# zpelgrims/pota

Hardware: AMD Instinct MI355X
Metric: bidir redistribution Msamples/s at 4K, double-gauss 50mm (higher is better)
Workload: dtype f64

## Files before the change

pota_amd/csrc/lentil_device.h:

```cpp
#pragma once
#include <hip/hip_runtime.h>
#include <stdint.h>

#include "../../include/lentil_hip.h"

#define LD_DEV __device__ __forceinline__

namespace lentil {

constexpr float kAiPi = 3.14159265358979323846f;
constexpr float kAiPiOver2 = 1.57079632679489661923f;
constexpr float kAiEpsilon = 1.0e-4f;
constexpr float kAiInfinite = 1.0e30f;
constexpr double kPi = 3.14159265358979323846;

enum PolyId {
  P_OUT_X = 0, P_OUT_Y, P_OUT_DX, P_OUT_DY, P_OUT_T,
  P_AP_X, P_AP_Y, P_AP_DX, P_AP_DY,
  P_DAP_00, P_DAP_01, P_DAP_10, P_DAP_11,
  P_DOUT_00, P_DOUT_01, P_DOUT_10, P_DOUT_11,
  P_DAPPOS_00, P_DAPPOS_01, P_DAPPOS_10, P_DAPPOS_11,
  P_COUNT
};

// ... 220 lines not shown
  ody = vx * ey0 + vy * ey1 + vz * ey2;
}

LD_DEV double ipow_u(double x, uint32_t e) {
  uint32_t odd = 0, n = 0;
  while (e > 2) { odd = (odd << 1) | (e & 1u); ++n; e >>= 1; }
  double p = (e == 2) ? x * x : x;
  for (uint32_t i = 0; i < n; ++i) {
    p = (odd & 1u) ? (x * p) * p : p * p;
    odd >>= 1;
  }
  return p;
}

struct LdsLens {
  const DevTerm *terms;
  const DevLens *k;

  LD_DEV double eval(int pid, const double v[4]) const {
    const uint32_t first = k->first[pid], count = k->count[pid];
    double sum = 0.0;
    for (uint32_t i = 0; i < count; ++i) {
      const DevTerm t = terms[first + i];
      const uint32_t e = __builtin_amdgcn_readfirstlane(t.e);
      double term = t.c;
#pragma unroll
      for (int var = 0; var < 4; ++var) {
        const uint32_t ev = (e >> (4 * var)) & 15u;
        if (ev == 1) term = term * v[var];
        else if (ev > 1) term = term * ipow_u(v[var], ev);
      }
      const uint32_t el = (e >> 16) & 15u;
      if (el) term = term * k->lambda_pow[el];
      sum = (i == 0) ? term : sum + term;
    }
    return sum;
  }

  LD_DEV void eval_bw(const double v[4], double pred_ap[2], double Jap[4], double out[4], double Jout[4]) const {
    pred_ap[0] = eval(P_AP_X, v);
    pred_ap[1] = eval(P_AP_Y, v);
    Jap[0] = eval(P_DAP_00, v); Jap[1] = eval(P_DAP_01, v);
    Jap[2] = eval(P_DAP_10, v); Jap[3] = eval(P_DAP_11, v);
    out[0] = eval(P_OUT_X, v); out[1] = eval(P_OUT_Y, v);
    out[2] = eval(P_OUT_DX, v); out[3] = eval(P_OUT_DY, v);
    Jout[0] = eval(P_DOUT_00, v); Jout[1] = eval(P_DOUT_01, v);
    Jout[2] = eval(P_DOUT_10, v); Jout[3] = eval(P_DOUT_11, v);
  }
  LD_DEV double transmittance(const double v[4]) const { return eval(P_OUT_T, v); }
  LD_DEV void eval_fw_newton(const double v[4], double pred_ap[2], double pred_dir[2], double Jap[4], double Jappos[4]) const {
    pred_ap[0] = eval(P_AP_X, v); pred_ap[1] = eval(P_AP_Y, v);
    pred_dir[0] = eval(P_AP_DX, v); pred_dir[1] = eval(P_AP_DY, v);
    Jap[0] = eval(P_DAP_00, v); Jappos[0] = eval(P_DAPPOS_00, v);
    Jap[1] = eval(P_DAP_01, v); Jappos[1] = eval(P_DAPPOS_01, v);
    Jap[2] = eval(P_DAP_10, v); Jappos[2] = eval(P_DAPPOS_10, v);
    Jap[3] = eval(P_DAP_11, v); Jappos[3] = eval(P_DAPPOS_11, v);
  }
  LD_DEV void eval_out(const double v[4], double out[4]) const {
    out[0] = eval(P_OUT_X, v); out[1] = eval(P_OUT_Y, v);
    out[2] = eval(P_OUT_DX, v); out[3] = eval(P_OUT_DY, v);
  }
  LD_DEV const DevLens &consts() const { return *k; }
};

struct NewtonState {
  double x, y, dx, dy;
  double sqr_err, sqr_ap_err;
  double out[4];
  int k, error;
};

LD_DEV void newton_init(NewtonState &s) {
  s.x = 0; s.y = 0; s.dx = 0; s.dy = 0;
  s.sqr_err = 1e30; s.sqr_ap_err = 1e30;
  s.out[0] = s.out[1] = s.out[2] = s.out[3] = 0.0;
  s.k = 0; s.error = 0;
}

LD_DEV bool newton_continue(const NewtonState &s) {
  const double eps = 1e-8;
  return s.k < 100 && (s.sqr_err > eps || s.sqr_ap_err > eps) && s.error == 0;
}

template <class Lens>
LD_DEV void newton_iter(const Lens &L, const double scene[3], double ap_x, double ap_y, NewtonState &s) {
  const DevLens &k = L.consts();
  const double R = k.outer_pupil_curvature_radius;
  const double prev_sqr_err = s.sqr_err, prev_sqr_ap_err = s.sqr_ap_err;
  const double begin[4] = {s.x, s.y, s.dx, s.dy};
  double pred_ap[2], Jap[4], Jout[4];
  L.eval_bw(begin, pred_ap, Jap, s.out, Jout);
  const double d0 = ap_x - pred_ap[0], d1 = ap_y - pred_ap[1];
  s.sqr_ap_err = d0 * d0 + d1 * d1;
  {
    const double invdet = 1.0 / (Jap[0] * Jap[3] - Jap[1] * Jap[2]);
    const double i00 = Jap[3] * invdet, i11 = Jap[0] * invdet;
    const double i01 = -Jap[1] * invdet, i10 = -Jap[2] * invdet;
    s.dx += i00 * d0; s.dy += i10 * d0;
    s.dx += i01 * d1; s.dy += i11 * d1;
  }
  double pos[3], dir[3];
  double on_dx, on_dy;
  if (k.outer_pupil_geometry == LENTIL_GEOM_SPHERICAL) {
    sphereToCs(s.out[0], s.out[1], s.out[2], s.out[3], pos, dir, -R, R);
    double vx = scene[0] - pos[0], vy = scene[1] - pos[1], vz = scene[2] - pos[2];
    normalise3(vx, vy, vz);
    csToSphere(pos, vx, vy, vz, on_dx, on_dy, -R, R);
  } else {
    const bool cy = k.outer_pupil_geometry == LENTIL_GEOM_CYL_Y;
    cylinderToCs(s.out[0], s.out[1], s.out[2], s.out[3], pos, dir, -R, R, cy);
    double vx = scene[0] - pos[0], vy = scene[1] - pos[1], vz = scene[2] - pos[2];
    normalise3(vx, vy, vz);
    csToCylinder(pos, vx, vy, vz, on_dx, on_dy, -R, R, cy);
  }
  const double e0 = on_dx - s.out[2], e1 = on_dy - s.out[3];
  s.sqr_err = e0 * e0 + e1 * e1;
  {
    const double invdet = 1.0 / (Jout[0] * Jout[3] - Jout[1] * Jout[2]);
    const double i00 = Jout[3] * invdet, i11 = Jout[0] * invdet;
    const double i01 = -Jout[1] * invdet, i10 = -Jout[2] * invdet;
    s.x += 0.72 * i00 * e0; s.y += 0.72 * i10 * e0;
    s.x += 0.72 * i01 * e1; s.y += 0.72 * i11 * e1;
  }
  int error = s.error;
  if (s.sqr_err > prev_sqr_err) error |= 1;
  if (s.sqr_ap_err > prev_sqr_ap_err) error |= 2;
  if (s.out[0] != s.out[0]) error |= 4;
  if (s.out[2] * s.out[2] + s.out[3] * s.out[3] > 1.0) error |= 8;
  if (s.k < 10) error = 0;
  s.error = error;
  s.k += 1;
}

template <class Lens>
LD_DEV double lens_evaluate(const Lens &L, const double in[4], double out[4]) {
  L.eval_out(in, out);
  return fmax(0.0, L.transmittance(in));
}

template <class Lens>
LD_DEV void lens_pt_sample_aperture(const Lens &L, double in[4], double ap_x, double ap_y, double dist,
                                    double &out_dx, double &out_dy) {
  double dx = in[2], dy = in[3];
  double pred_dx = 0.0, pred_dy = 0.0;
  double sqr_err = 3.4028234663852886e38;
  for (int k = 0; k < 5 && sqr_err > 1e-4; ++k) {
    const double begin[4] = {in[0] + dist * dx, in[1] + dist * dy, dx, dy};
    double pred[2], pred_dir[2], Jap[4], Jappos[4];
    L.eval_fw_newton(begin, pred, pred_dir, Jap, Jappos);
    const double pred_x = pred[0], pred_y = pred[1];
    pred_dx = pred_dir[0];
    pred_dy = pred_dir[1];
    const double j00 = Jap[0] + dist * Jappos[0];
    const double j01 = Jap[1] + dist * Jappos[1];
    const double j10 = Jap[2] + dist * Jappos[2];
    const double j11 = Jap[3] + dist * Jappos[3];
    const double invdet = 1.0 / (j00 * j11 - j01 * j10);
    const double i00 = j11 * invdet, i11 = j00 * invdet, i01 = -j01 * invdet, i10 = -j10 * invdet;
    const double r0 = ap_x - pred_x, r1 = ap_y - pred_y;
    dx += i00 * r0; dy += i10 * r0;
    dx += i01 * r1; dy += i11 * r1;
    sqr_err = r0 * r0 + r1 * r1;
  }
  out_dx = pred_dx; out_dy = pred_dy;
  in[2] = dx; in[3] = dy;
}

LD_DEV double y0_plane_z(const double pos[3], const double dir[3]) {
  const double n = sqrt(dir[0] * dir[0] + dir[1] * dir[1] + dir[2] * dir[2]);
  const double dy = dir[1] / n, dz = dir[2] / n;
  return pos[2] + (dz * (0.0 - pos[1])) / dy;
}

template <class Lens>
LD_DEV double camera_get_y0_intersection_distance(const Lens &L, double sensor_shift, double aperture_housing_radius,
                                                  double sensor_out[4], double out[4], double &transmittance) {
  const DevLens &k = L.consts();
  double sensor[4] = {0.0, 0.0, 0.0, 0.0};
  double adx, ady;
  lens_pt_sample_aperture(L, sensor, 0.0, aperture_housing_radius * 0.25, sensor_shift, adx, ady);
  sensor[0] += sensor[2] * sensor_shift;
  sensor[1] += sensor[3] * sensor_shift;
  transmittance = lens_evaluate(L, sensor, out);
  for (int c = 0; c < 4; ++c) sensor_out[c] = sensor[c];
  const double R = k.outer_pupil_curvature_radius;
  double pos[3], dir[3];
  if (k.outer_pupil_geometry == LENTIL_GEOM_SPHERICAL) sphereToCs(out[0], out[1], out[2], out[3], pos, dir, -R, R);
  else cylinderToCs(out[0], out[1], out[2], out[3], pos, dir, -R, R, k.outer_pupil_geometry == LENTIL_GEOM_CYL_Y);
  return y0_plane_z(pos, dir);
}

template <class Lens>
LD_DEV double newton_finish(const Lens &L, const NewtonState &s, double &out4) {
  const DevLens &k = L.consts();
  int error = s.error;
  if (s.out[0] * s.out[0] + s.out[1] * s.out[1] > k.outer_pupil_radius * k.outer_pupil_radius) error |= 16;
  if (error == 0) {
    const double begin[4] = {s.x, s.y, s.dx, s.dy};
    out4 = L.transmittance(begin);
  } else {
    out4 = 0.0;
  }
  return fmax(0.0, out4);
}

template <class Lens>
LD_DEV double lt_sample_aperture(const Lens &L, const double scene[3], double ap_x, double ap_y,
                                 double sensor[4], double out[5], int *iters = nullptr) {
  NewtonState s;
  newton_init(s);
  while (newton_continue(s)) newton_iter(L, scene, ap_x, ap_y, s);
  const double T = newton_finish(L, s, out[4]);
  out[0] = s.out[0]; out[1] = s.out[1]; out[2] = s.out[2]; out[3] = s.out[3];
  if (iters) *iters = s.k;
// ... 466 lines not shown
```

pota_amd/csrc/lentil_hip.hip:

```cpp
#include <hip/hip_runtime.h>
#include <hip/hip_ext.h>

#include <algorithm>
#include <atomic>
#include <chrono>
#include <cmath>
#include <cstdio>
#include <cstdlib>
#include <cstring>
#include <deque>
#include <mutex>
#include <new>
#include <string>
#include <vector>

#include "lentil_kernels.h"
#include "lentil_closest_replay.h"
#include "lentil_tl_chroma_mgpu.h"
#include "lentil_lens_jit.h"
#include "lentil_camera_rays.h"
#include "lentil_trace_points.h"
#include "lentil_list_draws.h"
#include "generated/embedded_sources.inc"

// ... 2615 lines not shown
    const int rc = redistribute_streamed(ctx, &streamed, &deferred);
    if (rc) return rc;
    if (ctx->stall_redo) return LENTIL_OK;
  }
  if (!streamed) { const int rc = join_clear(ctx); if (rc) return rc; }
  if (!streamed && ctx->V.n) {
    ScanPlan plan;
    {
      const int rc = plan_scan(ctx, plan);
      if (rc) return rc;
    }
    const uint32_t M = plan.M;
    for (int ci = 0; ci < C; ++ci) {
      lentil_hip_ctx::Chunk &ch = ctx->chunks[ci];
      if (M) {
        auto bound = [&](int i) -> uint64_t {
          if (i <= 0) return 0;
          if (i >= C) return plan.n_tiles;
          const double f0 = C > 1 ? ctx->first_chunk_frac : 1.0;
          const double x = f0 + (1.0 - f0) * (double)(i - 1) / (double)(C - 1);
          const uint64_t b = (uint64_t)((double)plan.n_tiles * x);
          return b > plan.n_tiles ? plan.n_tiles : b;
        };
        ch.tile_begin = bound(ci);
        ch.tile_end = bound(ci + 1);
        ch.v_begin = ch.tile_begin * plan.sa.ppt * M;
        ch.v_end = ch.tile_end * plan.sa.ppt * M;
        if (ch.v_begin > ctx->V.n) ch.v_begin = ctx->V.n;
        if (ch.v_end > ctx->V.n) ch.v_end = ctx->V.n;
      } else {
        ch.v_begin = ((ctx->V.n * ci / C) + 63) & ~63ull;
        ch.v_end = ci == C - 1 ? ctx->V.n : (((ctx->V.n * (ci + 1) / C) + 63) & ~63ull);
        if (ch.v_begin > ctx->V.n) ch.v_begin = ctx->V.n;
        if (ch.v_end > ctx->V.n) ch.v_end = ctx->V.n;
      }
      if (ch.v_end > ch.v_begin) {
        const int rc = launch_scan(ctx, plan, ch, ctx->d_ctr + ci);
        if (rc) return rc;
        ++ctx->last_scan_launches;
      }
      HIP_TRY(ctx, hipEventRecord(ch.scanned, ctx->stream));
    }
  }
  if (!streamed) {
    HIP_TRY(ctx, hipEventRecord(ctx->ev[1], ctx->stream));
    HIP_TRY(ctx, hipEventRecord(ctx->scans_done, ctx->stream));
  }
  if (!streamed && ctx->V.n) {
    DrawArgs da{};
    init_draw_args(ctx, da);
    const int forced_rounds = forced_blind_rounds();
    const int blind_rounds = forced_rounds ? forced_rounds : 3;
    std::vector<int> rounds_of(C, blind_rounds);
    std::vector<DrawArgs> das(C, da);
    std::vector<char> enq(C, 0);
    for (int ci = 0; ci < C; ++ci) {
      HIP_TRY(ctx, hipStreamWaitEvent(ctx->chunks[ci].stream, ctx->chunks[ci].scanned, 0));
      bool done = false;
      if (!forced_rounds && ctx->chunks[ci].have_est) {
        const int r = ctx->chunks[ci].est_rounds;
        rounds_of[ci] = r < 2 ? 2 : (r > 6 ? 6 : r);
      }
      const int rc = enqueue_chunk_draws_blind(ctx, ci, das[ci], rounds_of[ci], &done);
      if (rc) return rc;
      enq[ci] = done ? 1 : 0;
      if (done) ++ctx->last_blind;
    }
    for (int ci = 0; ci < C; ++ci) {
      if (enq[ci]) continue;
      const int rc = enqueue_chunk_draws(ctx, ci, das[ci], blind_rounds);
      if (rc) return rc;
    }
    bool any_blind = false;
    for (int ci = 0; ci < C; ++ci) any_blind = any_blind || enq[ci];
    if (any_blind)
      for (int ci = 0; ci < C; ++ci)
        HIP_TRY(ctx, hipMemcpyAsync(ctx->h_ctr_pinned + ci, ctx->d_ctr + ci, sizeof(DevCounters), hipMemcpyDeviceToHost, ctx->chunks[ci].stream));
    if (any_blind) {
      for (int ci = 0; ci < C; ++ci) HIP_TRY(ctx, hipStreamSynchronize(ctx->chunks[ci].stream));
      ctx->h_ctr.assign(ctx->h_ctr_pinned, ctx->h_ctr_pinned + C);
      ctx->h_ctr_valid = true;
      unsigned long long it = 0, tr = 0, sl = 0;
      for (const DevCounters &k : ctx->h_ctr) { it += k.newton_iters; tr += k.tries; sl += k.slow_solves; }
      if (tr) { ctx->mean_iters = (double)it / (double)tr; ctx->parked_frac = (double)sl / (double)tr; }
    }
    for (int ci = 0; ci < C; ++ci) {
      lentil_hip_ctx::Chunk &ch = ctx->chunks[ci];
      if (!enq[ci]) continue;
      const DevCounters c = ctx->h_ctr[(size_t)ci];
      if (c.fallback) {
        ctx->h_ctr_valid = false;
        if (c.fallback & 64ull) {
          char note[256];
          snprintf(note, sizeof note, "chunk %d: a list of %u occlusion probes did not fit its buffers (%llu): the chunk's draws were redone with counted lists",
                   ci, c.probe_max, (unsigned long long)ch.probe_cap_now);
          ctx->redo_note = note;
          if (c.rounds_used) {
            probe_abandon(ctx);
            return fail(ctx, LENTIL_ERR_NOMEM, "occlusion probes: a list of " + std::to_string(c.probe_max) + " segments in a later round did not fit buffers capped at " +
                                                   std::to_string(ch.probe_cap_now) + ": the frame is incomplete");
          }
          ch.probe_counted = true;
          ch.pb.occ_dirty = true;
          ctx->n_dev_overflows += c.probe_over;
          HIP_TRY(ctx, hipMemsetAsync((char *)(ctx->d_ctr + ci) + offsetof(DevCounters, probe_n), 0, offsetof(DevCounters, reserved_) - offsetof(DevCounters, probe_n), ch.stream));
        }
        ++ctx->last_fallback;
        HIP_TRY(ctx, hipMemsetAsync((char *)(ctx->d_ctr + ci) + offsetof(DevCounters, n_tasks), 0,
                                    offsetof(DevCounters, inv_row_min) - offsetof(DevCounters, n_tasks), ch.stream));
        HIP_TRY(ctx, hipMemsetAsync((char *)(ctx->d_ctr + ci) + offsetof(DevCounters, fallback), 0, sizeof(unsigned long long), ch.stream));
        const int rc = enqueue_chunk_draws(ctx, ci, das[ci], blind_rounds);
        if (rc) return rc;
        rounds_of[ci] = blind_rounds;
      } else {
        const uint64_t cap = ch.v_end - ch.v_begin;
        ch.est_items = c.work_count < cap ? c.work_count : cap;
        ch.est_sum = c.sum_samples;
        ch.est_rounds = (int)c.rounds_used;
        if (ch.est_items == 0 || c.n_active[rounds_of[ci] & 1] == 0) ch.n_items = 0;
      }
    }
    int max_rounds = ctx->last_rounds;
    for (int ci = 0; ci < C; ++ci) if (rounds_of[ci] > max_rounds) max_rounds = rounds_of[ci];
    for (int ci = 0; ci < C; ++ci) {
      lentil_hip_ctx::Chunk &ch = ctx->chunks[ci];
      HIP_TRY(ctx, hipStreamSynchronize(ch.stream));
      if (ch.n_items == 0) continue;
      ctx->h_ctr_valid = false;
      int rounds = rounds_of[ci];
      const int rc = finish_rounds(ctx, ci, das[ci], rounds_of[ci], &rounds);
      if (rounds > ch.est_rounds) ch.est_rounds = rounds;
      if (rc) return rc;
      if (rounds > max_rounds) max_rounds = rounds;
    }
    ctx->last_rounds = max_rounds;
    {
      uint64_t items = 0, sum = 0;
      int rounds = 0;
      bool all = true;
      for (const auto &ch : ctx->chunks) {
        all = all && ch.have_est;
        items += ch.est_items; sum += ch.est_sum;
        if (ch.est_rounds > rounds) rounds = ch.est_rounds;
      }
      if (all) { ctx->have_total_est = true; ctx->est_items_total = items; ctx->est_sum_total = sum; ctx->est_rounds_total = rounds; }
    }
  }
  if (ctx->F.zkey_dbg && ctx->V.n && !ctx->closest_deferred) {
    hipLaunchKernelGGL(debug_gather_kernel, dim3((unsigned)ctx->num_cu * 8), dim3(256), 0, ctx->stream, ctx->F, ctx->V, P,
                       ctx->have_lens ? ctx->hlens.length : 0.0);
    HIP_TRY(ctx, hipGetLastError());
  }
  if (ctx->F.zkey && ctx->V.n && !ctx->closest_deferred) {
    hipLaunchKernelGGL(closest_gather_kernel, dim3((unsigned)ctx->num_cu * 8), dim3(256), 0, ctx->stream, ctx->F, ctx->V);
    HIP_TRY(ctx, hipGetLastError());
  }
  if (ctx->early_resolve_pending) {
    ctx->early_resolve_pending = false;
    if (ctx->F.dir && ctx->F.touched && !ctx->last_fallback) {
      if (!ctx->late_resolve_done) {
        HIP_TRY(ctx, hipStreamWaitEvent(ctx->stream, ctx->ev_res, 0));
        const int rc = launch_resolve_half(ctx, ctx->stream, 2u);
        if (rc) return rc;
      }
      ctx->resolved_valid = true;
    } else {
      HIP_TRY(ctx, hipStreamWaitEvent(ctx->stream, ctx->ev_res, 0));
// ... 1125 lines not shown
```

pota_amd/csrc/lentil_kernels.h:

```cpp
#pragma once
#include "lentil_device.h"
#include "lentil_batch_model.h"
#include "generated/lens_registry.h"

using namespace lentil;

struct DevCounters {
  unsigned long long work_count;
  unsigned long long sum_samples;
  unsigned long long redistributed;
  unsigned long long attempted;
  unsigned long long accepted;
  unsigned long long overflow;
  unsigned long long log_count;
  unsigned long long newton_iters;
  unsigned long long tries;
  unsigned long long lane_rounds;
  unsigned long long slow_solves;
  unsigned long long fallback;
  unsigned long long rounds_used;
  unsigned int n_tasks[2];
  unsigned int task_head[2];
  unsigned int n_active[2];
  unsigned int active_head[2];
// ... 1807 lines not shown
      k.count = ((count - t * 64u) < 64u ? (count - t * 64u) : 64u) | (c << 8);
      a.tasks[par][tb + c * nt + t] = k;
    }
  }
  return true;
}

LD_DEV void reset_round(DevCounters *c, uint32_t par) {
  c->n_tasks[par] = 0; c->task_head[par] = 0; c->n_active[par] = 0; c->active_head[par] = 0;
  c->pool_used[par] = 0;
  c->n_slow[par] = 0; c->slow_head[par] = 0; c->waves_done[par] = 0; c->waves_started[par] = 0; c->accept_done[par] = 0;
  c->accept_items_done[par] = 0; c->accept_final[par] = 0;
}
__global__ void reset_round_kernel(DevCounters *c, uint32_t par, uint32_t keep_pool) {
  LENTIL_TL_SPAN(SPAN_RESET);
  const unsigned long long used = c->pool_used[par];
  reset_round(c, par);
  if (keep_pool) c->pool_used[par] = used;
}

__global__ __launch_bounds__(256) void prep_items_kernel(DrawArgs a) {
  const uint64_t i = (uint64_t)blockIdx.x * blockDim.x + threadIdx.x;
  uint64_t n_items = a.n_items;
  const unsigned long long sum_samples = a.ctr->sum_samples;
  if (a.blind) {
    const unsigned long long wc = a.ctr->work_count;
    const uint64_t n = wc < a.work_cap ? wc : a.work_cap;
    const uint64_t nch = (uint64_t)a.n_channels;
    const uint64_t units = nch * (4ull * sum_samples + (uint64_t)(3 * a.retries + 32) * n);
    const uint64_t tasks = units / 64 + 2 * n + 64;
    if (n > a.n_items || units > a.pool_cap || tasks > a.task_cap) {
      if (i == 0) { a.ctr->fallback = 32ull; a.ctr->n_active[0] = 0u; }
      return;
    }
    n_items = n;
  }
  if (i == 0) a.ctr->n_active[0] = (unsigned int)n_items;
  if (i >= n_items) return;
  const uint32_t item = (uint32_t)i;
  const ItemVisit h = load_item_visit(a, item, a.lens ? a.lens->length : 0.0);
  const ItemHdr hd = make_item_hdr(a.P, h.I.cs, h.px, h.py);
  a.hdr[item] = hd;
  const uint32_t samples = h.samples, max_total = samples * 5u;
  const uint32_t m_limit = max_total + (uint32_t)a.retries;
  uint32_t m_hi = samples + (uint32_t)a.retries;
  if (sum_samples < a.extra_below) m_hi += (uint32_t)(((unsigned long long)samples * a.extra_num) >> 8) + a.extra_const;
  if (m_hi > m_limit) m_hi = m_limit;
  ItemProg pg{};
  pg.m_lo = 0;
  pg.m_hi = m_hi;
  uint32_t off = 0;
  if (!emit_tasks(a, 0u, item, 0u, m_hi, off)) pg.m_hi = 0;
  pg.res_off = off;
  a.prog[item] = pg;
  a.active[0][item] = item;
}

template <class LensT>
LD_DEV uint32_t solve_result(const lentil_params &P, const LensT &L, const NewtonState &s) {
  const DevLens &k = L.consts();
  double out4;
  const float transmittance = (float)newton_finish(L, s, out4);
  if (transmittance <= 0) return kCodeFail;
  const double ipx = s.x + s.dx * k.back_focal_length;
  const double ipy = s.y + s.dy * k.back_focal_length;
  if (ipx * ipx + ipy * ipy > k.inner_pupil_radius * k.inner_pupil_radius) return kCodeFail;
  const double sx = s.x + s.dx * -P.sensor_shift;
  const double sy = s.y + s.dy * -P.sensor_shift;
  uint32_t pix;
  return po_sensor_to_pixel(P, sx, sy, pix) ? pix : kCodeOut;
}

#ifndef LENTIL_SOLVE_ATTR
#define LENTIL_SOLVE_ATTR __attribute__((amdgpu_waves_per_eu(3)))
#endif
template <class LensT, bool kTables, bool kChroma = false, bool kStream = false>
__global__ __launch_bounds__(256) LENTIL_SOLVE_ATTR void solve_po_kernel(DrawArgs a) {
  LENTIL_TL_SPAN(a.round == 0 ? SPAN_SOLVE_R0 : (a.round == 1 ? SPAN_SOLVE_R1 : SPAN_SOLVE_R2));
  __shared__ DevTerm s_terms[kTables ? kMaxTerms : 1];
  __shared__ DevLens s_k;
  __shared__ DevLens s_kc[kChroma ? 3 : 1];
  __shared__ float s_cdfRow[kMaxBokehRows];
  __shared__ uint64_t s_hdr[4][4];
  __shared__ double s_ap[4][64][2];
  __shared__ double s_fin[4][6][64];
  __shared__ uint32_t s_fin_err[4][64], s_fin_res[4][64];
  if (kTables) {
    const uint32_t nt = a.lens->n_terms;
    for (uint32_t i = threadIdx.x; i < nt; i += blockDim.x) s_terms[i] = a.terms[i];
  }
  if (threadIdx.x == 0) s_k = *a.lens;
  if (kChroma && threadIdx.x < 3) {
    DevLens h = *a.lens;
    const double lam = a.lambda[threadIdx.x];
    h.lambda_pow[0] = 1.0; h.lambda_pow[1] = lam;
    for (uint32_t e = 2; e <= kMaxExp; ++e) h.lambda_pow[e] = ipow_u(lam, e);
    s_kc[threadIdx.x] = h;
  }
  const bool row_in_lds = a.P.bokeh_enable_image && a.bokeh.y <= kMaxBokehRows;
  if (row_in_lds)
    for (int i = threadIdx.x; i < a.bokeh.y; i += blockDim.x) s_cdfRow[i] = a.bokeh.cdfRow[i];
  __syncthreads();
  const float *cdfRow = row_in_lds ? s_cdfRow : a.bokeh.cdfRow;
  LensT L;
  if constexpr (kTables) { L.terms = s_terms; L.k = &s_k; } else { L.k = &s_k; }
  const DevLens &k = s_k;
  const lentil_params &P = a.P;

  if (blockIdx.x == 0 && threadIdx.x == 0 && !a.no_reset) reset_round(a.ctr, (uint32_t)a.parity ^ 1u);
  const uint32_t par = (uint32_t)a.parity;
  const Task *tasks = a.tasks[par];
  uint32_t *res = a.pool[par];
  uint32_t n_tasks = 0;
  if constexpr (!kStream) n_tasks = a.ctr->n_tasks[par] < a.task_cap ? a.ctr->n_tasks[par] : a.task_cap;
  const uint32_t lane = lane_id();
  const unsigned long long lt_mask = (1ull << lane) - 1ull;
  if (a.slow_live && a.slow && lane == 0) atomicAdd(&a.ctr->waves_started[par], 1u);
#ifdef LENTIL_PROBE_BUILD
  if (kStream && a.dispatch_probe && a.round == 1 && lane == 0) atomicAdd(&a.ctr->probe_res_xcc[0][xcc_id()], 1u);
#endif

  uint32_t cur_item = 0, cur_m = 0, cur_res = 0, cur_left = 0, cur_chan = 0;
  (void)cur_chan;
  bool no_more = false;
  constexpr uint32_t kNoTicket = 0xFFFFFFFFu;
  uint32_t ticket = kNoTicket, polls = 0;
  uint64_t ticket_t0 = 0;
  uint32_t idle_naps = 1u;
  (void)ticket; (void)polls; (void)ticket_t0; (void)idle_naps;
  bool busy = false;
  uint32_t res_idx = 0, cur_chan_lane = 0, my_item = 0;
  (void)cur_chan_lane;
  const uint32_t wv = threadIdx.x >> 6;
  uint32_t cur_pos = 0;
  uint32_t fin_n = 0;
  auto flush_finished = [&]() {
    if (fin_n == 0u) return;
    __builtin_amdgcn_fence(__ATOMIC_RELEASE, "wavefront", "local");
    __builtin_amdgcn_wave_barrier();
    __builtin_amdgcn_fence(__ATOMIC_ACQUIRE, "wavefront", "local");
    if (lane < fin_n) {
      NewtonState t;
      t.x = s_fin[wv][0][lane]; t.y = s_fin[wv][1][lane]; t.dx = s_fin[wv][2][lane]; t.dy = s_fin[wv][3][lane];
      t.out[0] = s_fin[wv][4][lane]; t.out[1] = s_fin[wv][5][lane]; t.out[2] = 0.0; t.out[3] = 0.0;
      t.sqr_err = 0.0; t.sqr_ap_err = 0.0; t.k = 0;
      const uint32_t ew = s_fin_err[wv][lane];
      t.error = (int)(ew & 0xFFu);
      LensT Lf = L;
      if constexpr (kChroma) Lf.k = &s_kc[(ew >> 8) & 3u];
      res[s_fin_res[wv][lane]] = solve_result(P, Lf, t);
    }
    __builtin_amdgcn_fence(__ATOMIC_RELEASE, "wavefront", "local");
    __builtin_amdgcn_wave_barrier();
    fin_n = 0u;
  };
  auto start_task = [&]() {
    cur_pos = 0u;
    __builtin_amdgcn_fence(__ATOMIC_RELEASE, "wavefront", "local");
    __builtin_amdgcn_wave_barrier();
    __builtin_amdgcn_fence(__ATOMIC_ACQUIRE, "wavefront", "local");
    if (lane < cur_left) {
      double ax = 0.0, ay = 0.0;
      po_aperture_sample(P, a.bokeh, cdfRow, (uint32_t)s_hdr[wv][3], cur_m + lane, ax, ay);
      s_ap[wv][lane][0] = ax; s_ap[wv][lane][1] = ay;
    }
    __builtin_amdgcn_fence(__ATOMIC_RELEASE, "wavefront", "local");
    __builtin_amdgcn_wave_barrier();
    __builtin_amdgcn_fence(__ATOMIC_ACQUIRE, "wavefront", "local");
  };
  double target[3] = {0, 0, 1};
  double ap_x = 0.0, ap_y = 0.0;
  NewtonState s;
  newton_init(s);
  uint32_t st_iters = 0, st_tries = 0, st_rounds = 0;
  const bool parking = a.slow != nullptr && a.round >= a.slow_from_round && (kStream || a.ctr->sum_samples < a.slow_below);
  bool producers_gone = false;
  (void)producers_gone;

  while (true) {
    const unsigned long long busy_mask = __ballot(busy);
    const uint32_t inflight = (uint32_t)__builtin_popcountll(busy_mask);
    const uint32_t n_idle = 64u - inflight;
    const uint32_t my_rank = (uint32_t)__builtin_popcountll(~busy_mask & lt_mask);
    uint32_t filled = 0;
    while (filled < n_idle) {
      if (cur_left == 0) {
        if (no_more) break;
        if constexpr (kStream) {
          if (ticket == kNoTicket) {
            uint32_t q = 0;
            if (lane == 0) q = atomicAdd(&a.ctr->task_head[par], 1u);
            ticket = __builtin_amdgcn_readfirstlane(q);
            polls = 0;
            ticket_t0 = __builtin_amdgcn_s_memrealtime();
          }
          if (ticket >= a.task_cap) { no_more = true; break; }
          uint64_t w1 = 0;
          if (lane == 0) w1 = ld_coherent64(reinterpret_cast<const uint64_t *>(tasks + ticket) + 1);
          const uint32_t w1_hi = __builtin_amdgcn_readfirstlane((uint32_t)(w1 >> 32));
          if ((w1_hi >> kTaskTagShift) != a.epoch) {
            if (lane == 0) tl_add(TL_POLLS_EMPTY, 1u);
            if (__builtin_amdgcn_s_memrealtime() - ticket_t0 > (a.stuck_ticks ? a.stuck_ticks : kStuckTicks)) {
              if (lane == 0 && atomicCAS(&a.ctr->stuck, 0u, 2u | (ticket << 2)) == 0u) {
                unsigned int *si = a.ctr->stuck_info;
                si[0] = (uint32_t)a.round; si[1] = par; si[2] = ld_coherent32(&a.ctr->n_tasks[par]);
                si[3] = ld_coherent32(&a.ctr->accept_done[0]); si[4] = ld_coherent32(&a.ctr->accept_started[0]);
                si[5] = w1_hi; si[6] = blockIdx.x; si[7] = ld_coherent32(&a.ctr->task_head[par]);
              }
              no_more = true;
            }
            break;
          }
          if ((w1_hi & 0xFFu) == kEndCount) {
            no_more = true;
            break;
          }
          uint64_t w0 = 0;
          if (lane == 0) w0 = ld_coherent64(reinterpret_cast<const uint64_t *>(tasks + ticket));
          cur_item = __builtin_amdgcn_readfirstlane((uint32_t)w0);
          cur_m = __builtin_amdgcn_readfirstlane((uint32_t)(w0 >> 32));
          cur_res = __builtin_amdgcn_readfirstlane((uint32_t)w1);
          cur_left = w1_hi & 0xFFu;
          if (kChroma) cur_chan = (w1_hi >> 8) & 3u;
          ticket = kNoTicket;
          if (lane == 0) tl_add(TL_TASKS_TAKEN, 1u);
          if (cur_left) {
            if (lane < 4u) {
              const uint64_t *hp = reinterpret_cast<const uint64_t *>(a.hdr + cur_item);
              s_hdr[wv][lane] = ld_coherent64(hp + lane);
            }
            start_task();
          }
          if (cur_left == 0) continue;
        } else {
          uint32_t q = 0;
          if (lane == 0) q = atomicAdd(&a.ctr->task_head[par], 1u);
          q = __builtin_amdgcn_readfirstlane(q);
          if (q >= n_tasks) { no_more = true; break; }
          const Task t = tasks[q];
          cur_item = __builtin_amdgcn_readfirstlane(t.item);
          cur_m = __builtin_amdgcn_readfirstlane(t.m_base);
          cur_res = __builtin_amdgcn_readfirstlane(t.res_off);
          cur_left = __builtin_amdgcn_readfirstlane(t.count) & 0xFFu;
          if (kChroma) cur_chan = (__builtin_amdgcn_readfirstlane(t.count) >> 8) & 3u;
          if (cur_left) {
            if (lane < 4u) s_hdr[wv][lane] = reinterpret_cast<const uint64_t *>(a.hdr + cur_item)[lane];
            start_task();
          }
          if (cur_left == 0) continue;
        }
      }
      uint32_t take = n_idle - filled;
      if (take > cur_left) take = cur_left;
      if (!busy && my_rank >= filled && my_rank < filled + take) {
        const uint32_t j = my_rank - filled;
        res_idx = cur_res + j;
        const uint64_t *hs = s_hdr[wv];
        target[0] = __longlong_as_double((long long)hs[0]);
        target[1] = __longlong_as_double((long long)hs[1]);
        target[2] = __longlong_as_double((long long)hs[2]);
        ap_x = s_ap[wv][cur_pos + j][0];
        ap_y = s_ap[wv][cur_pos + j][1];
        newton_init(s);
        ++st_tries;
        busy = true;
        my_item = cur_item;
        if constexpr (kChroma) { L.k = &s_kc[cur_chan]; cur_chan_lane = cur_chan; }
      }
      cur_pos += take; cur_res += take; cur_left -= take; filled += take;
    }
    if (inflight + filled == 0u) {
      flush_finished();
      if (!kStream || no_more) break;
      for (uint32_t i = 0; i < idle_naps; ++i) __builtin_amdgcn_s_sleep(127);
      if (idle_naps < 8u) idle_naps <<= 1;
      continue;
    }
    idle_naps = 1u;

    if (busy) { newton_iter(L, target, ap_x, ap_y, s); ++st_iters; }
    ++st_rounds;
#ifdef LENTIL_TIMELINE
    { const uint32_t nb_ = (uint32_t)__builtin_popcountll(__ballot(busy)); if (lane == 0) tl_add(!kStream || a.round ? TL_ITERS_LATER : (a.instance ? TL_ITERS_B : TL_ITERS_A), nb_); }
#endif

    {
      const bool fin = busy && !newton_continue(s);
      const unsigned long long fmask = __ballot(fin);
      if (fmask) {
        const uint32_t nfin = (uint32_t)__builtin_popcountll(fmask);
        if (fin_n + nfin > 64u) flush_finished();
        if (fin) {
          const uint32_t q = fin_n + (uint32_t)__builtin_popcountll(fmask & lt_mask);
          s_fin[wv][0][q] = s.x; s_fin[wv][1][q] = s.y; s_fin[wv][2][q] = s.dx; s_fin[wv][3][q] = s.dy;
          s_fin[wv][4][q] = s.out[0]; s_fin[wv][5][q] = s.out[1];
          s_fin_err[wv][q] = ((uint32_t)s.error & 0xFFu) | ((kChroma ? cur_chan_lane : 0u) << 8);
          s_fin_res[wv][q] = res_idx;
          busy = false;
        }
        fin_n += nfin;
      }
    }
    if (kStream && a.slow_after_producers && !producers_gone && (st_rounds & 15u) == 0u) {
      uint32_t pd = 0;
      if (lane == 0) pd = ld_coherent32(a.producers_done);
      producers_gone = (uint32_t)__builtin_amdgcn_readfirstlane(pd) >= a.producers_total;
    }
    if (parking && (!kStream || !a.slow_after_producers || producers_gone || no_more) &&
        ((a.slow_live && !a.slow_dry_only) || (no_more && __builtin_popcountll(__ballot(busy)) <= a.slow_max_lanes))) {
      const bool park = busy && s.k >= a.slow_at;
      const unsigned long long pmask = __ballot(park);
      if (pmask) {
        const uint32_t sq = slow_queue(a);
        uint32_t base = 0;
        if (lane == (uint32_t)__builtin_ctzll(pmask)) base = atomicAdd(&a.ctr->n_slow[sq], (uint32_t)__builtin_popcountll(pmask));
        base = __shfl(base, __builtin_ctzll(pmask));
        const uint32_t slot = base + (uint32_t)__builtin_popcountll(pmask & lt_mask);
        if (park && pmask && slot < a.slow_cap) {
          tl_add(TL_PARKED, 1u);
          double *d = reinterpret_cast<double *>(a.slow + slot);
          const uint32_t chan_word = (kChroma ? cur_chan_lane : 0u) | (par ? kSlowParBit : 0u) |
                                     ((a.slow_live && a.slow_indirect) ? kSlowIndirectBit : 0u);
          if (a.slow_live) {
            const double pay[11] = {target[0], target[1], target[2], ap_x, ap_y, s.x, s.y, s.dx, s.dy, s.sqr_err, s.sqr_ap_err};
#pragma unroll
            for (int i = 0; i < 11; ++i) st_agent64(d + i, (uint64_t)__double_as_longlong(pay[i]));
            st_agent64(d + 11, (uint64_t)(uint32_t)s.k | ((uint64_t)(uint32_t)s.error << 32));
            st_agent64(d + 12, (uint64_t)res_idx | ((uint64_t)chan_word << 32));
            if (a.item_ready && a.slow_indirect) {
              st_agent64(d + 13, (uint64_t)my_item << 32);
              atomicAdd(&a.hdr[my_item].parked, 1u);
            }
            if (a.slow_indirect) st_agent32(res + res_idx, kCodePendingBase | slot);
            asm volatile("s_waitcnt vmcnt(0)" ::: "memory");
            st_agent64(d + 15, slow_tag(a, kSlowRecord));
          } else {
            d[0] = target[0]; d[1] = target[1]; d[2] = target[2]; d[3] = ap_x; d[4] = ap_y;
            d[5] = s.x; d[6] = s.y; d[7] = s.dx; d[8] = s.dy; d[9] = s.sqr_err; d[10] = s.sqr_ap_err;
            uint32_t *u = reinterpret_cast<uint32_t *>(d + 11);
            u[0] = (uint32_t)s.k; u[1] = (uint32_t)s.error; u[2] = res_idx; u[3] = chan_word;
          }
          busy = false;
        }
      }
    }
  }
  flush_finished();
#ifdef LENTIL_PROBE_BUILD
  if (kStream && a.dispatch_probe && a.round == 1 && lane == 0) atomicSub(&a.ctr->probe_res_xcc[0][xcc_id()], 1u);
#endif
  if (a.slow_live && a.slow && a.slow_close) {
    asm volatile("s_waitcnt vmcnt(0)" ::: "memory");
    uint32_t close = 0;
    if (lane == 0) {
      const uint32_t done = atomicAdd(&a.ctr->waves_done[par], 1u) + 1u;
      const uint32_t begun = ld_coherent32(&a.ctr->waves_started[par]);
      const uint32_t taken = ld_coherent32(&a.ctr->task_head[par]);
      const uint32_t published = kStream ? ld_coherent32(&a.ctr->n_tasks[par]) : n_tasks;
      const bool complete = !kStream || ld_coherent32(a.producers_done) >= a.producers_total;
      close = (done == begun && complete && taken >= published) ? 1u : 0u;
    }
    if (__builtin_amdgcn_readfirstlane(close)) {
      uint32_t n = ld_coherent32(&a.ctr->n_slow[slow_queue(a)]);
// ... 2077 lines not shown
```

pota_amd/csrc/lentil_stream_pass.h:

```cpp
#pragma once


static int streamed_finish(lentil_hip_ctx *ctx, StreamTail &t, const DevCounters *pinned, bool can_fix, bool *streamed) {
  const int C = ctx->n_chunks;
  lentil_hip_ctx::Chunk &ch = ctx->chunks[0];
  int rc;
  ctx->h_ctr.assign(pinned, pinned + C);
  ctx->h_ctr_valid = true;
  ctx->last_streamed = 1;
  const DevCounters c = ctx->h_ctr[0];
  ch.was_blind = true;
  if (c.probe_snap[0]) {
    char buf[640];
    int n = snprintf(buf, sizeof buf, "[probe] epoch %u: accept blocks begun %u of %u when the last item was done; per XCD begun:", ctx->epoch, c.probe_snap[33], c.probe_snap[34]);
    for (int x = 0; x < 8; ++x) n += snprintf(buf + n, sizeof buf - n, " %u", c.probe_snap[1 + x]);
    const char *kinds[3] = {"second round's solve waves resident", "second round's straggler waves resident", "first round's straggler waves resident"};
    for (int k = 0; k < 3; ++k) {
      n += snprintf(buf + n, sizeof buf - n, " | %s:", kinds[k]);
      for (int x = 0; x < 8; ++x) n += snprintf(buf + n, sizeof buf - n, " %u", c.probe_snap[9 + 8 * k + x]);
    }
    fprintf(stderr, "%s\n", buf);
  }
  if (c.fallback || c.stuck) {
    char note[768];
// ... 11 lines not shown
    ctx->redo_note = note;
    if (c.stuck && (c.stuck & 3u) == 1u && ctx->d_ranges) {
      const uint32_t tk = c.stuck >> 2;
      uint64_t w[4] = {0, 0, 0, 0};
      if ((uint64_t)tk + 2 < ctx->range_cap)
        (void)hipMemcpy(w, ctx->d_ranges + (tk ? tk - 1 : 0), sizeof w, hipMemcpyDeviceToHost);
      char more[256];
      snprintf(more, sizeof more, " | range slots from %u on (host read-back): %016llx %016llx %016llx %016llx, range_head %u",
               tk ? tk - 1 : 0, (unsigned long long)w[0], (unsigned long long)w[1], (unsigned long long)w[2], (unsigned long long)w[3], c.range_head);
      ctx->redo_note += more;
    }
    if (getenv("LENTIL_STREAM_DEBUG")) {
      fprintf(stderr, "[stream] note: %s\n", ctx->redo_note.c_str());
      fprintf(stderr, "[stream] redo: who %u ticket %u epoch %u range_head %u pubs_done %u scan_done %u | fallback %llu stuck %u | items %llu (cap %u) tasks %u (cap %u) pool %llu (cap %llu) ranges %u (cap %u)\n",
              c.stuck & 3u, c.stuck >> 2, ctx->epoch, c.range_head, c.publishers_done, c.scan_blocks_done, c.fallback, c.stuck, c.work_count, t.item_cap, c.n_tasks[0], t.task_cap, c.pool_used[0], (unsigned long long)t.pool_cap,
              c.n_ranges, t.range_cap);
      HIP_TRY(ctx, hipEventRecord(ctx->ev[2], ctx->stream));
      HIP_TRY(ctx, hipEventSynchronize(ctx->ev[2]));
      float ms_scan = 0.f, ms_all = 0.f;
      (void)hipEventElapsedTime(&ms_scan, ctx->ev[0], ctx->ev[1]);
      (void)hipEventElapsedTime(&ms_all, ctx->ev[0], ctx->ev[2]);
      fprintf(stderr, "[stream] scan %.3f ms, pass until the read-back %.3f ms\n", ms_scan, ms_all);
      fprintf(stderr, "[stream] queues: n_tasks %u/%u task_head %u/%u n_active %u/%u active_head %u/%u accept_done %u/%u pool_used %llu/%llu\n",
              c.n_tasks[0], c.n_tasks[1], c.task_head[0], c.task_head[1], c.n_active[0], c.n_active[1], c.active_head[0], c.active_head[1],
              c.accept_done[0], c.accept_done[1], c.pool_used[0], c.pool_used[1]);
      fprintf(stderr, "[stream] stragglers: live %d waves_done %u/%u (round 1: %u) parked %u/%u heads %u/%u cap %u waves %u rounds_used %llu\n", (int)t.live,
              c.waves_done[0], c.waves_started[0], c.waves_done[1], c.n_slow[0], c.n_slow[1], c.slow_head[0], c.slow_head[1],
              t.da.slow_cap, t.da.slow_waves, c.rounds_used);
    }
    if (c.stuck) {
      g_stat_stuck.fetch_add(1, std::memory_order_relaxed);
      if (t.inject) g_stat_stuck_injected.fetch_add(1, std::memory_order_relaxed);
      else {
        std::lock_guard<std::mutex> lock(g_stall_notes_mutex);
        if (g_stall_notes.size() < 8) g_stall_notes.push_back(ctx->redo_note + (t.deferred ? " | end deferred" : " | end awaited") + (can_fix ? "" : ", abandoned") +
                                                              " | frame " + std::to_string(ctx->P.xres) + "x" + std::to_string(ctx->P.yres) + ", " + std::to_string(ctx->V.n) + " visits");
      }
    }
    if (ctx->notes.size() < 8) ctx->notes.push_back(ctx->redo_note);
    if (!can_fix) {
      if (c.stuck) ++ctx->n_stuck;
      ++ctx->last_fallback;
      ++ctx->totals.abandoned_incomplete;
      ctx->last_rounds = (int)c.rounds_used;
      if (!c.stuck) {
        const uint64_t n_items = c.work_count < ctx->V.n ? c.work_count : ctx->V.n;
        ctx->have_total_est = true;
        ctx->est_items_total = n_items; ctx->est_sum_total = c.sum_samples;
      }
      for (int ci = 0; ci < C; ++ci) ctx->chunks[ci].have_est = false;
      *streamed = true;
      return LENTIL_OK;
    }
    t.did_more = true;
    if (c.stuck && c.rounds_used) {
      ++ctx->n_stuck;
      ctx->stall_redo = true;
      ctx->h_ctr_valid = false;
      ctx->late_resolve_done = false;
      *streamed = true;
      return LENTIL_OK;
    }
    if (c.stuck) {
      ++ctx->n_stuck;
      HIP_TRY(ctx, hipMemsetAsync((char *)ctx->d_ctr + offsetof(DevCounters, stuck), 0, sizeof(unsigned int), ch.stream));
    }
    ctx->h_ctr_valid = false;
    ctx->late_resolve_done = false;
    ++ctx->last_fallback;
    HIP_TRY(ctx, hipMemsetAsync((char *)ctx->d_ctr + offsetof(DevCounters, n_tasks), 0,
                                offsetof(DevCounters, inv_row_min) - offsetof(DevCounters, n_tasks), ch.stream));
    HIP_TRY(ctx, hipMemsetAsync((char *)ctx->d_ctr + offsetof(DevCounters, fallback), 0, sizeof(unsigned long long), ch.stream));
    DrawArgs db{};
    init_draw_args(ctx, db);
    if ((rc = enqueue_chunk_draws(ctx, 0, db, 3))) return rc;
    HIP_TRY(ctx, hipStreamSynchronize(ch.stream));
    int rounds = 3;
    if (ch.n_items) { if ((rc = finish_rounds(ctx, 0, db, 3, &rounds))) return rc; }
    ch.est_rounds = rounds;
    ctx->last_rounds = rounds;
  } else {
    const uint64_t n_items = c.work_count < ctx->V.n ? c.work_count : ctx->V.n;
    ch.have_est = true; ch.est_items = n_items; ch.est_sum = c.sum_samples; ch.est_rounds = (int)c.rounds_used;
    if (c.tries) { ctx->mean_iters = (double)c.newton_iters / (double)c.tries; ctx->parked_frac = (double)c.slow_solves / (double)c.tries; }
    int rounds = t.blind_rounds;
    if (t.lean) ++ctx->n_lean;
    const bool short_after_all = t.predicted && n_items && (c.n_tasks[1] != 0u || (t.lean && c.n_active[t.blind_rounds & 1] != 0u));
    const bool open_end = n_items && ((t.lean && c.n_tasks[1] != 0u) || c.n_active[t.blind_rounds & 1] != 0);
    if (open_end && !can_fix) {
      ++ctx->totals.abandoned_incomplete;
      if (ctx->notes.size() < 8) ctx->notes.push_back("abandoned before its end was looked at: the first accept had scheduled another round (lean tail's bet lost)");
    } else if (open_end) {
      t.did_more = true;
    }
    if (short_after_all) {
      ctx->bm_since_loss = 0;
      if (ctx->bm_margin16 >= 4u) ctx->lean_ok = false;
      else ctx->bm_margin16 += 1u;
    }
    if (t.predicted && !short_after_all && ++ctx->bm_since_loss >= 16u && ctx->bm_margin16 > 0u) { --ctx->bm_margin16; ctx->bm_since_loss = 0; }
    if (!can_fix && open_end) {
      if (t.lean) ++ctx->n_lean_lost;
      rounds = (int)c.rounds_used + 1;
    } else
    if (t.lean && n_items && c.n_tasks[1] != 0u) {
      ctx->h_ctr_valid = false;
      ctx->late_resolve_done = false;
      t.da.parity = 1; t.da.round = 1;
      t.da.producers_done = nullptr; t.da.producers_total = 0;
      t.da.slow_live = 0; t.da.slow_indirect = 0; t.da.slow_q = -1; t.da.slow_round = -1; t.da.slow_close = 1;
      t.da.emit_live = 0; t.da.lean_gate = 0; t.da.no_reset = 1;
      {
        DrawArgs dr = t.da;
        if (dr.slow) { dr.slow = t.slow_base + t.slow_cap_all / 2u; dr.slow_cap = t.slow_cap_all - t.slow_cap_all / 2u; }
        launch_solve(ctx, dr, ch.stream, (unsigned)ctx->num_cu);
      }
      hipLaunchKernelGGL(reset_round_kernel, dim3(1), dim3(1), 0, ch.stream, ctx->d_ctr, 0u, 1u);
      hipLaunchKernelGGL(accept_kernel<2>, dim3(t.accept_blocks), dim3(256), 0, ch.stream, t.da);
      HIP_TRY(ctx, hipGetLastError());
      t.da.no_reset = 0;
      if ((rc = finish_rounds(ctx, 0, t.da, 2, &rounds))) return rc;
      if (rounds > ch.est_rounds) ch.est_rounds = rounds;
      ++ctx->n_lean_lost;
    } else
    if (n_items && c.n_active[t.blind_rounds & 1] != 0) {
      ctx->h_ctr_valid = false;
      ctx->late_resolve_done = false;
      if ((rc = finish_rounds(ctx, 0, t.da, t.blind_rounds, &rounds))) return rc;
      if (rounds > ch.est_rounds) ch.est_rounds = rounds;
      if (t.lean) ++ctx->n_lean_lost;
    } else if (t.lean) {
      rounds = 1;
    }
    ctx->last_rounds = rounds;
  }
  ctx->have_total_est = true;
  ctx->est_items_total = ch.est_items; ctx->est_sum_total = ch.est_sum; ctx->est_rounds_total = ch.est_rounds;
  for (int ci = 0; ci < C; ++ci) ctx->chunks[ci].have_est = false;
  *streamed = true;
  return LENTIL_OK;
}

static bool stream_pass_applies(lentil_hip_ctx *ctx, DeviceTurn &turn, DrawArgs &da, uint64_t &items, uint64_t &units) {
  const lentil_params &P = ctx->P;
  if (!ctx->stream_mode || P.cameraType != LENTIL_POLYNOMIAL_OPTICS || !ctx->have_total_est || ctx->V.n == 0)
    return false;
  if (ctx->V.n > 0xFFFFFFF0ull) return false;
  if (no_tries(P)) return false;
  if (probing(ctx)) return false;
  if (!ctx->cleared_since_pass) return false;
  if (ctx->n_stuck >= (ctx->streams_concurrent ? 3u : 1u)) return false;
  {
    const uint64_t by_visits = ctx->stream_below_set ? 0ull : ctx->V.n / 24ull;
    if (ctx->est_sum_total >= (ctx->stream_below > by_visits ? ctx->stream_below : by_visits)) return false;
  }
  if (ctx->V.n_extra && !dma_multi_applies(ctx)) return false;
  if (ctx->V.n_extra && !fits_cu_beside_solves(dma_multi_lds(ctx), 1u, solve_block_lds(ctx), 512u)) return false;
  static const bool wait_for_turn = getenv("LENTIL_STREAM_WAIT") && getenv("LENTIL_STREAM_WAIT")[0] == '1';
  if (!turn.take(wait_for_turn)) return false;
  init_draw_args(ctx, da);
  ++ctx->n_streamed;
  g_stat_streamed.fetch_add(1, std::memory_order_relaxed);
  da.inject_stall = (ctx->inject_stall_at > 0 && ctx->n_streamed == (uint64_t)ctx->inject_stall_at) ? 1 : 0;
  items = 2 * ctx->est_items_total + 4096;
  if (items > ctx->V.n) items = ctx->V.n;
  units = chunk_units(P, (uint64_t)da.n_channels, 2 * ctx->est_sum_total + (1ull << 20), items);
  return units <= ctx->max_pool_units;
// ... 446 lines not shown
```

Baseline: 41690.

## Precompute Newton first iteration from origin once per block and share per wave

The first Newton iteration always starts at the zero state, so the backward polynomial evaluation and its Jacobian inverse are the same for every sample. This computes them once per block (per chroma channel) into shared memory. The pupil half-step, which depends only on the scene target, runs once per wave header. Each new sample then seeds its state from these shared values, skipping one full polynomial evaluation. Host iteration-count statistics are adjusted to include the skipped first iteration.

```diff
diff --git a/pota_amd/csrc/lentil_device.h b/pota_amd/csrc/lentil_device.h
--- a/pota_amd/csrc/lentil_device.h
+++ b/pota_amd/csrc/lentil_device.h
@@ -326,23 +326,26 @@
   return s.k < 100 && (s.sqr_err > eps || s.sqr_ap_err > eps) && s.error == 0;
 }
 
-template <class Lens>
-LD_DEV void newton_iter(const Lens &L, const double scene[3], double ap_x, double ap_y, NewtonState &s) {
-  const DevLens &k = L.consts();
-  const double R = k.outer_pupil_curvature_radius;
-  const double prev_sqr_err = s.sqr_err, prev_sqr_ap_err = s.sqr_ap_err;
-  const double begin[4] = {s.x, s.y, s.dx, s.dy};
-  double pred_ap[2], Jap[4], Jout[4];
-  L.eval_bw(begin, pred_ap, Jap, s.out, Jout);
+LD_DEV void newton_ap_inverse(const double Jap[4], double inv[4]) {
+  const double invdet = 1.0 / (Jap[0] * Jap[3] - Jap[1] * Jap[2]);
+  inv[0] = Jap[3] * invdet; inv[3] = Jap[0] * invdet;
+  inv[1] = -Jap[1] * invdet; inv[2] = -Jap[2] * invdet;
+}
+LD_DEV void newton_ap_step(const double pred_ap[2], const double inv[4], double ap_x, double ap_y, NewtonState &s) {
   const double d0 = ap_x - pred_ap[0], d1 = ap_y - pred_ap[1];
   s.sqr_ap_err = d0 * d0 + d1 * d1;
-  {
-    const double invdet = 1.0 / (Jap[0] * Jap[3] - Jap[1] * Jap[2]);
-    const double i00 = Jap[3] * invdet, i11 = Jap[0] * invdet;
-    const double i01 = -Jap[1] * invdet, i10 = -Jap[2] * invdet;
-    s.dx += i00 * d0; s.dy += i10 * d0;
-    s.dx += i01 * d1; s.dy += i11 * d1;
-  }
+  s.dx += inv[0] * d0; s.dy += inv[2] * d0;
+  s.dx += inv[1] * d1; s.dy += inv[3] * d1;
+}
+LD_DEV void newton_ap_half(const double pred_ap[2], const double Jap[4], double ap_x, double ap_y, NewtonState &s) {
+  double inv[4];
+  newton_ap_inverse(Jap, inv);
+  newton_ap_step(pred_ap, inv, ap_x, ap_y, s);
+}
+
+LD_DEV void newton_pupil_half(const DevLens &k, const double Jout[4], const double scene[3], double prev_sqr_err,
+                              double prev_sqr_ap_err, NewtonState &s) {
+  const double R = k.outer_pupil_curvature_radius;
   double pos[3], dir[3];
   double on_dx, on_dy;
   if (k.outer_pupil_geometry == LENTIL_GEOM_SPHERICAL) {
@@ -374,6 +377,43 @@
   if (s.k < 10) error = 0;
   s.error = error;
   s.k += 1;
+}
+
+template <class Lens>
+LD_DEV void newton_iter(const Lens &L, const double scene[3], double ap_x, double ap_y, NewtonState &s) {
+  const double prev_sqr_err = s.sqr_err, prev_sqr_ap_err = s.sqr_ap_err;
+  const double begin[4] = {s.x, s.y, s.dx, s.dy};
+  double pred_ap[2], Jap[4], Jout[4];
+  L.eval_bw(begin, pred_ap, Jap, s.out, Jout);
+  newton_ap_half(pred_ap, Jap, ap_x, ap_y, s);
+  newton_pupil_half(L.consts(), Jout, scene, prev_sqr_err, prev_sqr_ap_err, s);
+}
+
+struct NewtonOrigin {
+  double pred_ap[2], Jap_inv[4], out[4], Jout[4];
+};
+
+template <class Lens>
+LD_DEV void newton_origin(const Lens &L, NewtonOrigin &o) {
+  const double begin[4] = {0.0, 0.0, 0.0, 0.0};
+  double Jap[4];
+  L.eval_bw(begin, o.pred_ap, Jap, o.out, o.Jout);
+  newton_ap_inverse(Jap, o.Jap_inv);
+}
+
+LD_DEV void newton_first_ap(const NewtonOrigin &o, double ap_x, double ap_y, NewtonState &s) {
+  newton_ap_step(o.pred_ap, o.Jap_inv, ap_x, ap_y, s);
+}
+LD_DEV void newton_first_pupil(const DevLens &k, const NewtonOrigin &o, const double scene[3], NewtonState &s) {
+  s.out[0] = o.out[0]; s.out[1] = o.out[1]; s.out[2] = o.out[2]; s.out[3] = o.out[3];
+  newton_pupil_half(k, o.Jout, scene, s.sqr_err, s.sqr_ap_err, s);
+}
+LD_DEV void newton_first(const DevLens &k, const NewtonOrigin &o, const double scene[3], double ap_x, double ap_y,
+                         NewtonState &s) {
+  const double prev_sqr_ap_err = s.sqr_ap_err;
+  newton_first_ap(o, ap_x, ap_y, s);
+  s.out[0] = o.out[0]; s.out[1] = o.out[1]; s.out[2] = o.out[2]; s.out[3] = o.out[3];
+  newton_pupil_half(k, o.Jout, scene, s.sqr_err, prev_sqr_ap_err, s);
 }
 
 template <class Lens>
diff --git a/pota_amd/csrc/lentil_hip.hip b/pota_amd/csrc/lentil_hip.hip
--- a/pota_amd/csrc/lentil_hip.hip
+++ b/pota_amd/csrc/lentil_hip.hip
@@ -2721,7 +2721,7 @@
       ctx->h_ctr_valid = true;
       unsigned long long it = 0, tr = 0, sl = 0;
       for (const DevCounters &k : ctx->h_ctr) { it += k.newton_iters; tr += k.tries; sl += k.slow_solves; }
-      if (tr) { ctx->mean_iters = (double)it / (double)tr; ctx->parked_frac = (double)sl / (double)tr; }
+      if (tr) { ctx->mean_iters = (double)(it + tr) / (double)tr; ctx->parked_frac = (double)sl / (double)tr; }
     }
     for (int ci = 0; ci < C; ++ci) {
       lentil_hip_ctx::Chunk &ch = ctx->chunks[ci];
diff --git a/pota_amd/csrc/lentil_kernels.h b/pota_amd/csrc/lentil_kernels.h
--- a/pota_amd/csrc/lentil_kernels.h
+++ b/pota_amd/csrc/lentil_kernels.h
@@ -1913,6 +1913,8 @@
   __shared__ DevLens s_kc[kChroma ? 3 : 1];
   __shared__ float s_cdfRow[kMaxBokehRows];
   __shared__ uint64_t s_hdr[4][4];
+  __shared__ NewtonOrigin s_org[kChroma ? 3 : 1];
+  __shared__ double s_first[4][3];
   __shared__ double s_ap[4][64][2];
   __shared__ double s_fin[4][6][64];
   __shared__ uint32_t s_fin_err[4][64], s_fin_res[4][64];
@@ -1935,6 +1937,15 @@
   const float *cdfRow = row_in_lds ? s_cdfRow : a.bokeh.cdfRow;
   LensT L;
   if constexpr (kTables) { L.terms = s_terms; L.k = &s_k; } else { L.k = &s_k; }
+  {
+    const uint32_t c = (kChroma && threadIdx.x < 3u) ? threadIdx.x : 0u;
+    LensT Lo = L;
+    if constexpr (kChroma) Lo.k = &s_kc[c];
+    NewtonOrigin o;
+    newton_origin(Lo, o);
+    if (threadIdx.x < (kChroma ? 3u : 1u)) s_org[c] = o;
+  }
+  __syncthreads();
   const DevLens &k = s_k;
   const lentil_params &P = a.P;
 
@@ -1995,6 +2006,16 @@
       po_aperture_sample(P, a.bokeh, cdfRow, (uint32_t)s_hdr[wv][3], cur_m + lane, ax, ay);
       s_ap[wv][lane][0] = ax; s_ap[wv][lane][1] = ay;
     }
+    {
+      const uint64_t *hs = s_hdr[wv];
+      const double tg[3] = {__longlong_as_double((long long)hs[0]), __longlong_as_double((long long)hs[1]),
+                            __longlong_as_double((long long)hs[2])};
+      const uint32_t c = kChroma ? cur_chan : 0u;
+      NewtonState f;
+      newton_init(f);
+      newton_first_pupil(kChroma ? s_kc[c] : s_k, s_org[c], tg, f);
+      if (lane == 0u) { s_first[wv][0] = f.x; s_first[wv][1] = f.y; s_first[wv][2] = f.sqr_err; }
+    }
     __builtin_amdgcn_fence(__ATOMIC_RELEASE, "wavefront", "local");
     __builtin_amdgcn_wave_barrier();
     __builtin_amdgcn_fence(__ATOMIC_ACQUIRE, "wavefront", "local");
@@ -2014,6 +2035,7 @@
     const uint32_t n_idle = 64u - inflight;
     const uint32_t my_rank = (uint32_t)__builtin_popcountll(~busy_mask & lt_mask);
     uint32_t filled = 0;
+    bool ended_first = false;
     while (filled < n_idle) {
       if (cur_left == 0) {
         if (no_more) break;
@@ -2093,6 +2115,12 @@
         ap_x = s_ap[wv][cur_pos + j][0];
         ap_y = s_ap[wv][cur_pos + j][1];
         newton_init(s);
+        const NewtonOrigin &o = s_org[kChroma ? cur_chan : 0u];
+        newton_first_ap(o, ap_x, ap_y, s);
+        s.x = s_first[wv][0]; s.y = s_first[wv][1]; s.sqr_err = s_first[wv][2];
+        s.out[0] = o.out[0]; s.out[1] = o.out[1]; s.out[2] = o.out[2]; s.out[3] = o.out[3];
+        s.k = 1;
+        ended_first = !newton_continue(s);
         ++st_tries;
         busy = true;
         my_item = cur_item;
@@ -2109,7 +2137,7 @@
     }
     idle_naps = 1u;
 
-    if (busy) { newton_iter(L, target, ap_x, ap_y, s); ++st_iters; }
+    if (busy && !ended_first) { newton_iter(L, target, ap_x, ap_y, s); ++st_iters; }
     ++st_rounds;
 #ifdef LENTIL_TIMELINE
     { const uint32_t nb_ = (uint32_t)__builtin_popcountll(__ballot(busy)); if (lane == 0) tl_add(!kStream || a.round ? TL_ITERS_LATER : (a.instance ? TL_ITERS_B : TL_ITERS_A), nb_); }
diff --git a/pota_amd/csrc/lentil_stream_pass.h b/pota_amd/csrc/lentil_stream_pass.h
--- a/pota_amd/csrc/lentil_stream_pass.h
+++ b/pota_amd/csrc/lentil_stream_pass.h
@@ -117,7 +117,7 @@
   } else {
     const uint64_t n_items = c.work_count < ctx->V.n ? c.work_count : ctx->V.n;
     ch.have_est = true; ch.est_items = n_items; ch.est_sum = c.sum_samples; ch.est_rounds = (int)c.rounds_used;
-    if (c.tries) { ctx->mean_iters = (double)c.newton_iters / (double)c.tries; ctx->parked_frac = (double)c.slow_solves / (double)c.tries; }
+    if (c.tries) { ctx->mean_iters = (double)(c.newton_iters + c.tries) / (double)c.tries; ctx->parked_frac = (double)c.slow_solves / (double)c.tries; }
     int rounds = t.blind_rounds;
     if (t.lean) ++ctx->n_lean;
     const bool short_after_all = t.predicted && n_items && (c.n_tasks[1] != 0u || (t.lean && c.n_active[t.blind_rounds & 1] != 0u));
```

Result: faster. 43090, median of 6 (+3.4%).
